# tvlearn/evo

Measured on AMD Instinct MI355X. Metric: E-step candidate-state evals/sec (NxS), full EM iteration, higher is better.
Workload: dtype f64; 1 GPU; ES3C D=256 H=512 S=200 N=100k f64 (north-star shape); algo=es3c, N_total=100000, N_rank0=100000, D=256, H=512, S=200, step=10 full EM iterations, world_size_rccl=1, ea=fit/randflip 10 parents x 1 child x 1 gen, states=p_init_Kn=1/H (init_states default), rng=device, mstep=device, parallelism=dp1

## Files before the change

### evo_amd/csrc/common.hpp

```cpp
#pragma once
#include <hip/hip_runtime.h>
#include <stdint.h>

typedef unsigned long long u64;
typedef long long i64;

#define EVO_F64_MIN (-1.7976931348623157e308)
#define EVO_F64_TINY (2.2250738585072014e-308)
#define EVO_WAVE 64

#define EVO_ERR_BAD_ENTRY 8
#define EVO_ERR_LIST_FULL 16
__device__ __forceinline__ int guard_index(int v, long long bound, int *__restrict__ err) {
  if (v < 0 || (long long)v >= bound) {
    atomicOr(err, EVO_ERR_BAD_ENTRY);
    return 0;
  }
  return v;
}
#define EVO_FLAG_NAN 1u
#define EVO_FLAG_NEGINF 2u
#define EVO_FLAG_POSINF 4u

__device__ __forceinline__ int wave_id_uniform() {
  return __builtin_amdgcn_readfirstlane((int)(threadIdx.x >> 6));
}
__device__ __forceinline__ int lane_id() { return (int)(threadIdx.x & 63); }

template <int CTRL, int ROWMASK>
__device__ __forceinline__ double dpp_move(double v) {
  const int lo = __double2loint(v), hi = __double2hiint(v);
  const int lo2 = __builtin_amdgcn_update_dpp(lo, lo, CTRL, ROWMASK, 0xF, false);
  const int hi2 = __builtin_amdgcn_update_dpp(hi, hi, CTRL, ROWMASK, 0xF, false);
  return __hiloint2double(hi2, lo2);
}
__device__ __forceinline__ double lane63_f64(double v) {
  const int lo = __builtin_amdgcn_readlane(__double2loint(v), 63);
  const int hi = __builtin_amdgcn_readlane(__double2hiint(v), 63);
  return __hiloint2double(hi, lo);
}
__device__ __forceinline__ double wave_sum(double v) {
  v += dpp_move<0xB1, 0xF>(v);
  v += dpp_move<0x4E, 0xF>(v);
  v += dpp_move<0x141, 0xF>(v);
  v += dpp_move<0x140, 0xF>(v);
  {
    const double t = dpp_move<0x142, 0xA>(v);
    if ((lane_id() >> 4) & 1) v += t;
  }
  {
    const double t = dpp_move<0x143, 0xC>(v);
    if (lane_id() >= 32) v += t;
  }
  return lane63_f64(v);
}
__device__ __forceinline__ double wave_max(double v) {
  v = fmax(v, dpp_move<0xB1, 0xF>(v));
  v = fmax(v, dpp_move<0x4E, 0xF>(v));
  v = fmax(v, dpp_move<0x141, 0xF>(v));
  v = fmax(v, dpp_move<0x140, 0xF>(v));
  v = fmax(v, dpp_move<0x142, 0xA>(v));
  v = fmax(v, dpp_move<0x143, 0xC>(v));
  return lane63_f64(v);
}
__device__ __forceinline__ unsigned dpp_max_u32(unsigned v, unsigned o) { return v > o ? v : o; }
template <int CTRL, int ROWMASK>
__device__ __forceinline__ unsigned dpp_move_u32(unsigned v) {
  return (unsigned)__builtin_amdgcn_update_dpp((int)v, (int)v, CTRL, ROWMASK, 0xF, false);
}
__device__ __forceinline__ unsigned row16_max_u32(unsigned v) {
  v = dpp_max_u32(v, dpp_move_u32<0xB1, 0xF>(v));
  v = dpp_max_u32(v, dpp_move_u32<0x4E, 0xF>(v));
  v = dpp_max_u32(v, dpp_move_u32<0x141, 0xF>(v));
  v = dpp_max_u32(v, dpp_move_u32<0x140, 0xF>(v));
  return v;
}
__device__ __forceinline__ unsigned wave_max_u32(unsigned v) {
  v = row16_max_u32(v);
  v = dpp_max_u32(v, dpp_move_u32<0x142, 0xA>(v));
  v = dpp_max_u32(v, dpp_move_u32<0x143, 0xC>(v));
  return (unsigned)__builtin_amdgcn_readlane((int)v, 63);
}

__device__ __forceinline__ unsigned wave_min_u32(unsigned v) { return ~wave_max_u32(~v); }
__device__ __forceinline__ double wave_min(double v);

__device__ __forceinline__ int wave_sum_i(int v) {
#pragma unroll
  for (int o = 32; o > 0; o >>= 1) v += __shfl_xor(v, o, 64);
  return v;
}

__device__ __forceinline__ double clamp_lpj(double v, unsigned &flags) {
  if (v != v) {
    flags |= EVO_FLAG_NAN;
    return EVO_F64_MIN;
  }
  if (isinf(v)) {
    flags |= (v < 0.0) ? EVO_FLAG_NEGINF : EVO_FLAG_POSINF;
    return 0.0;
  }
  return v;
}

__device__ __forceinline__ int pop_msb(u64 &bits) {
  int b = __clzll((long long)bits);
  bits &= ~(0x8000000000000000ull >> b);
  return b;
}

__device__ __forceinline__ double ordered_strided_sum(const double *__restrict__ p, i64 stride, i64 count) {
  double s = 0.0;
  i64 b = 0;
  for (; b + 8 <= count; b += 8) {
    double v[8];
#pragma unroll
    for (int u = 0; u < 8; u++) v[u] = p[(b + u) * stride];
#pragma unroll
    for (int u = 0; u < 8; u++) s += v[u];
  }
  for (; b < count; b++) s += p[b * stride];
  return s;
}

__device__ __forceinline__ void lds_barrier() { asm volatile("s_waitcnt lgkmcnt(0)\n\ts_barrier" ::: "memory"); }
__device__ __forceinline__ void lds_wave_fence() { asm volatile("s_waitcnt lgkmcnt(0)" ::: "memory"); }

#define DIG_IDX_BITS 14
#define DIG_MAX_H (1 << DIG_IDX_BITS)
#define DIG_SLOTS 4
__device__ __forceinline__ void digest_add(u64 &d, int &k, int h) {
  if (k < DIG_SLOTS) d |= (u64)h << (8 + DIG_IDX_BITS * k);
  k++;
}
__device__ __forceinline__ u64 digest_close(u64 d, int k) { return d | (u64)(k < 255 ? k : 255); }
__device__ __forceinline__ int dig_k(u64 d) { return (int)(d & 0xFFull); }
__device__ __forceinline__ int dig_idx(u64 d, int j) {
  return (int)((d >> (8 + DIG_IDX_BITS * j)) & (u64)(DIG_MAX_H - 1));
}
__device__ __forceinline__ u64 make_digest(const u64 *sp, int HW) {
  u64 d = 0;
  int k = 0;
  for (int w0 = 0; w0 < HW; w0 += 8) {
    u64 wv[8];
#pragma unroll
    for (int u = 0; u < 8; u++) wv[u] = (w0 + u < HW) ? sp[w0 + u] : 0ull;
#pragma unroll
    for (int u = 0; u < 8; u++) {
      u64 bits = wv[u];
      while (bits) digest_add(d, k, (w0 + u) * 64 + pop_msb(bits));
    }
  }
  return digest_close(d, k);
}

__device__ __forceinline__ double fast_rcp(double d) {
  double r = __builtin_amdgcn_rcp(d);
  r = fma(fma(-d, r, 1.0), r, r);
  r = fma(fma(-d, r, 1.0), r, r);
  return r;
}

struct LogDetAcc {
  double m = 1.0;
  int e = 0;
  __device__ __forceinline__ void mul(double d) {
    int ex;
    const double f = frexp(fabs(d), &ex);
    m *= f;
    e += ex;
    if (m < 0x1p-500) {
      int e2;
      m = frexp(m, &e2);
      e += e2;
    }
  }
  __device__ __forceinline__ double value() const { return log(m) + (double)e * 0.6931471805599453094; }
};

__device__ __forceinline__ double wave_max_dpp(double v) { return wave_max(v); }
__device__ __forceinline__ double wave_min(double v) { return -wave_max(-v); }
```

### evo_amd/csrc/evo_amd.hip

```cpp
#include "../../include/evo_amd.h"

#include <dlfcn.h>
#include <math.h>
#include <stdarg.h>
#include <stdio.h>
#include <stdlib.h>
#include <string.h>

#include <atomic>
#include <chrono>
#include <memory>
#include <string>
#include <type_traits>
#include <vector>

#include "common.hpp"
#include "gemm_f64.hpp"
#include "kernels_bsc.hpp"
#include "kernels_common.hpp"
#include "kernels_evolve.hpp"
#include "kernels_mstep.hpp"
#include "kernels_sssc.hpp"
#include "kernels_sssc_quad.hpp"
#include "kernels_fused.hpp"
// ... 343 lines not shown
  DevBuf<double> Y, yy, y2sum;
  int ldY = 0;
  PinnedBuf<double> h_acc, h_par;
  PinnedBuf<double> h_theta;
  double *h_theta_dev = nullptr;
  bool h_theta_fresh = false;
  DevBuf<double> theta_bak;
  bool theta_bak_valid = false;
  unsigned long long mbox_seq = 0;
  DevBuf<unsigned> mbox_counter;
  PinnedBuf<int> h_err;
  DevBuf<u64> states, cand;
  DevBuf<u64> dig, cand_dig;
  DevBuf<double> lpj, cand_lpj;
  DevBuf<double> lpj_alt;
  DevBuf<int> cand_counts;
  DevBuf<u64> cand_raw, dupold;
  DevBuf<int> gen_start;
  DevBuf<unsigned> flags;
  DevBuf<double> rowmax, rowsum, partial, partial2, diag;
  DevBuf<uint8_t> stage;
  DevBuf<double> W, Wt, G, Psi, Bm, mus, pilbar_v;
  DevBuf<double2> GP;
  DevBuf<double4> DG;
  DevBuf<double4> D1;
  DevBuf<PairEntry> PT;
  DevBuf<double> pies;
  double *dpar = nullptr;
  PinnedBuf<double> h_dpar;
  DevBuf<double> colpart;
  DevBuf<double> gjwork;
  DevBuf<double> tmpA, tmpB, tmpC;
  double ljc = 0;
  double *acc = nullptr;
  i64 acc_n = 0;
  DevBuf<double> acc_base;
  i64 ovf_n = 0;
  DevBuf<double> Es_own;
  double *Es = nullptr;
  DevBuf<int> list1, list2, list3, list_n, err;
  DevBuf<int> clist, clist_n;
  size_t clist_words() const { return clist.size() / 3; }
  DevBuf<OvfRec> ovf_rec;
  unsigned long long kn_gen = 1, census_gen = 0;
  int census_opt = 1;
  int merge_small = 1;
  DevBuf<double2> kap, cand_kap;
  unsigned long long kap_gen = ~0ull, cand_kap_gen = ~0ull;
  bool kap_carry = false;
  int stats_kappa = 1;
  int kappa_min = 16384;
  int stats_flat = 0;
  int fused_opt = 0;
  DevBuf<double> rowF;
  DevBuf<int> rowcnt, defer;
  DevBuf<double> fpart;
  DevBuf<unsigned long long> fprof;
  bool last_estep_fused = false;
  bool reduce_pending = false;
  long fused_calls = 0, unfused_calls = 0;
  int debug_poison_list = 0;
  int debug_fail_stats = 0;
  int census_skip = 0;
  DevBuf<double> tmp_y, tmp_lpj;
  DevBuf<u64> tmp_states;
  DevBuf<double> exact_buf;
  DevBuf<double> patch_img, patch_Y;
  DevBuf<double> patch_V;
  DevBuf<double> pred_buf, pred_Wt;
  DevBuf<int> pred_status;
  i64 pred_N = 0;
  int pred_D = 0;
  DevBuf<int> ps_slot, ps_status;
  DevBuf<u64> ps_s;
  DevBuf<double> ps_z, ps_y;
  i64 ps_N = 0, ps_T = 0;
  int ps_D = 0, ps_H = 0, ps_keep = -1;
  DevBuf<double> lle_d, lle_keep_d, lle_rho;
  DevBuf<int> lle_i;
  DevBuf<unsigned> lle_flags;
  DevBuf<u64> lle_keep_s, lle_hash;
  DevBuf<uint8_t> lle_keep_in;
  i64 lle_N = 0, lle_T = 0;
  int lle_H = 0, lle_keep = -1;
  DevBuf<uint8_t> codes_buf;
  unsigned long long rows_kn_gen = 0;
  int codes_path = -1;
  int init_home = -1;
  DevBuf<u64> init_scratch;
  DevBuf<double2> seed_gpt;
  DevBuf<double> seed_rows;
  DevBuf<double> refine_trace, score_buf;
  DevBuf<double> sweep_d;
  DevBuf<int> sweep_i;
  DevBuf<double> swap_d;
  DevBuf<int> swap_i;
  DevBuf<u64> remap_states, remap_dig;
  DevBuf<int> remap_i;
  DevBuf<unsigned long long> remap_sum, map_counts;
  i64 remap_N = 0;
  int remap_S = 0, remap_H = 0;
  DevBuf<u64> resize_states, resize_dig;
  DevBuf<int> resize_src;
  i64 resize_N = 0;
  int resize_S = 0, resize_H = 0;
  unsigned long long lpj_kn_gen = 0;
// ... 414 lines not shown
#define OPT_BOOL(f) nullptr, &evoamd_ctx::f
static int opt_flag(int v) { return v != 0; }
static const OptionRow OPTIONS[] = {
    {"sssc_k8", OPT_INT(k8_mode), [](int v) { return v < 0 ? -1 : (int)(v != 0); }},
    {"ebsc_f32", OPT_BOOL(f32_opt), opt_flag},
    {"bsc_direct", OPT_BOOL(bsc_direct), opt_flag, 0, 0, nullptr, nullptr,
     on_option_changes_derived},
    {"reconstruct_in_stats", OPT_BOOL(rec_in_stats), opt_flag},
    {"codes_path", OPT_INT(codes_path), nullptr, -1, CODES_GMEM, nullptr, "codes_path: -1 (auto), 0 registers, 1 LDS, 2 global memory"},
    {"merge_select_fused", OPT_INT(merge_select_fused), opt_flag},
    {"prefetch_lpj", OPT_BOOL(prefetch_lpj), opt_flag},
    {"inverse_block", OPT_INT(spd_block), nullptr, 0, 0, [](int v) { return v == 0 || v == 16 || v == 32; },
     "inverse_block: 0 (auto), 16 or 32"},
    {"overlap_gemm", OPT_INT(overlap_gemm)},
    {"stats_stage", OPT_INT(stats_stage)},
    {"stats_waves", OPT_INT(stats_waves)},
    {"pair_bins", OPT_INT(pair_bins)},
    {"gemm_streamk", OPT_INT(gemm_streamk)},
    {"b_transposed", OPT_INT(b_tn_opt)},
    {"pair_bins_scale", OPT_INT(bins_scale), nullptr, 1, 64, nullptr, "pair_bins_scale: 1 .. 64"},
    {"pair_bins_nwg", OPT_INT(bins_nwg), nullptr, 0, 0, [](int v) { return v >= 256 && v <= 2048 && (v % 256) == 0; },
     "pair_bins_nwg: 256 .. 2048, multiple of 256"},
    {"pair_bins_auto", OPT_INT(bins_auto), opt_flag},
    {"pair_bins_min", OPT_INT(bins_min)},
    {"bsc_stats_wave", OPT_INT(bsc_wave_opt)},
    {"gemm_workspace", OPT_INT(gemm_ws_opt)},
    {"sssc_precision", OPT_INT(sssc_prec32), [](int v) { return (int)(v == 32); }, 0, 0, [](int v) { return v == 64 || v == 32; },
     "sssc_precision: 64 or 32"},
    {"lpj_main_unstaged", OPT_INT(main_unstaged), opt_flag},
    {"lpj_singular_screen", OPT_INT(sing_screen), nullptr, 0, 2, nullptr, "lpj_singular_screen: 0 (never), 1 (automatic) or 2 (always)"},
    {"gemm_grouped", OPT_INT(gemm_grouped), opt_flag},
    {"gemm_per_xcd", OPT_INT(gemm_per_xcd)},
    {"init_states_home", OPT_INT(init_home), nullptr, -1, 1, nullptr, "init_states_home: -1 (auto), 0 LDS, 1 global memory"},
    {"background_unit", OPT_INT(bg_unit), opt_flag},
    {"fold_clear", OPT_INT(fold_clear), opt_flag},
    {"early_fork", OPT_INT(early_fork)},
    {"merge_small_levels", OPT_INT(merge_small), opt_flag},
    {"stats_flat", OPT_INT(stats_flat), opt_flag},
    {"theta_copy_engine", OPT_INT(theta_copy_engine), opt_flag},
    {"census_lists", OPT_INT(census_opt), opt_flag},
    {"sk_spare", OPT_INT(sk_spare), nullptr, -1, 32, nullptr, "sk_spare: -1 (automatic) or 0 .. 32 workgroups per XCD"},
    {"stats_chunks", OPT_INT(stats_chunks), nullptr, 1, 16, nullptr, "stats_chunks: 1 .. 16"},
    {"mailbox_side_stream", OPT_INT(mbox_side), opt_flag},
    {"fused_estep", OPT_INT(fused_opt), nullptr, 0, 2, nullptr, "fused_estep: 0 (never), 1 (automatic) or 2 (whenever the shape allows it)"},
    {"debug_poison_list", OPT_INT(debug_poison_list), opt_flag},
    {"debug_fail_stats", OPT_INT(debug_fail_stats), opt_flag},
    {"state_digest", OPT_BOOL(use_digest), opt_flag},
    {"inverse_spd", OPT_BOOL(spd_inverse), opt_flag},
};
static const OptionRow OPTIONS_LATER[] = {
  {"stats_kappa", OPT_INT(stats_kappa), nullptr, 0, 2, nullptr, "stats_kappa: 0 (never), 1 (automatic) or 2 (wherever the shape allows it)"},
  {"stats_kappa_min", OPT_INT(kappa_min), nullptr, 0, 1 << 20, nullptr, "stats_kappa_min: 0 .. 1048576 (x 1024 resident states)"},
};
#undef OPT_INT
#undef OPT_BOOL

extern "C" int evoamd_set_option(evoamd_ctx *c, const char *name, int value) {
  REQUIRE(c && name, "bad arguments");
  on_option(c);
  std::vector<const OptionRow *> rows;
  for (const OptionRow &o : OPTIONS) rows.push_back(&o);
  for (const OptionRow &o : OPTIONS_LATER) rows.push_back(&o);
  for (const OptionRow *row : rows) {
    const OptionRow &o = *row;
    if (strcmp(name, o.name) != 0) continue;
    if (o.err && !(o.accepts ? o.accepts(value) : (value >= o.lo && value <= o.hi))) return fail(EVOAMD_E_INVALID, "%s", o.err);
    const int v = o.norm ? o.norm(value) : value;
    if (o.ifield) c->*o.ifield = v;
    else c->*o.bfield = v != 0;
    if (o.after) o.after(c);
    return 0;
  }
  return fail(EVOAMD_E_INVALID, "unknown option '%s'", name);
}

static int join_fork(evoamd_ctx *c);

extern "C" int evoamd_synchronize(evoamd_ctx *c) {
  REQUIRE(c, "ctx is NULL");
  TRY(join_fork(c));
  HIP_TRY(hipStreamSynchronize(c->stream));
  return 0;
}

static i64 acc_len(const evoamd_ctx *c) {
  const i64 H = c->H, D = c->D;
  return (c->model == EVOAMD_MODEL_BSC) ? H * D + H * H + H + 1 + 8 : 2 * H + 4 * H * H + D * H + D + 8;
}
struct AccLayout {
  i64 Wp, Wq, pies, sigma;
  i64 xs, xss, xsz, xszsz, s_sz, sz_sz, sWp, y2;
  i64 tail;
};
static AccLayout acc_layout(const evoamd_ctx *c) {
  AccLayout a = {};
  const i64 H = c->H, D = c->D;
  if (c->model == EVOAMD_MODEL_BSC) {
    a.Wp = 0;
    a.Wq = H * D;
    a.pies = a.Wq + H * H;
    a.sigma = a.pies + H;
    a.tail = a.sigma + 1;
  } else {
    a.xs = 0;
    a.xss = H;
    a.xsz = a.xss + H * H;
    a.xszsz = a.xsz + H;
    a.sWp = a.xszsz + H * H;
    a.s_sz = a.sWp + D * H;
    a.sz_sz = a.s_sz + H * H;
    a.y2 = a.sz_sz + H * H;
    a.tail = a.y2 + D;
  }
  return a;
}
// ... 1594 lines not shown

extern "C" int evoamd_lpj_single_masked(evoamd_ctx *c, const double *y, const uint8_t *x_infr,
                                        const uint8_t *states_bool, int C, double *lpj_out, int32_t *flags_out) {
  REQUIRE(x_infr, "x_infr is NULL");
  return lpj_single_impl(c, y, x_infr, states_bool, C, lpj_out, flags_out);
}

static int estep_select(evoamd_ctx *c, int Mprime, double *sums_out) {
  on_kn_changed(c, KN_BY_SELECTION);
  {
    SpanGuard g(c, KID_VARY_KN);
    int *cl_n = census_mode(c) ? c->clist_n : nullptr;
    const i64 zero_n = c->fold_clear ? (i64)(c->ovf_n + c->acc_n) : 0;
    if (!c->fold_clear) cl_n = nullptr;
    const bool kap_carry = c->kap_carry && c->kap && c->cand_kap;
    with_spl(c->S, [&](auto spl) {
      with_cpl(c->Cmax, [&](auto cpl) {
        vary_kn_kernel<decltype(spl)::value, decltype(cpl)::value><<<cdiv(c->N, 4), 256, 0, c->stream>>>(
            c->states, c->lpj, c->cand, c->cand_lpj, c->cand_counts, c->N, c->S, c->S_perm, c->HW, c->Cmax, Mprime, c->rowmax,
            c->rowsum, c->partial, c->list_n, 4 * LIST_SHARDS, c->dig, c->cand_dig, (c->use_digest && c->dig) ? 1 : 0,
            c->pending_skip, c->err, cl_n, 4 * LIST_SHARDS, c->census_skip, c->acc_base, zero_n,
            kap_carry ? c->kap.get() : nullptr, kap_carry ? c->cand_kap.get() : nullptr);
      });
    });
    reduce3_partials_kernel<<<1, R3_THREADS, 0, c->stream>>>(c->partial, cdiv(c->N, 4), c->dpar);
    HIP_TRY(hipGetLastError());
    DBG_SYNC(c, "vary_kn");
    made_selection(c, cl_n != nullptr, zero_n > 0, kap_carry);
  }
  if (sums_out) {
    HIP_TRY(hipMemcpyAsync(sums_out, c->dpar + DP_ECNT0, 2 * sizeof(double), hipMemcpyDeviceToHost, c->stream));
    HIP_TRY(hipStreamSynchronize(c->stream));
  }
  return 0;
}

extern "C" int evoamd_vary_kn(evoamd_ctx *c, int Mprime, double *sums_out) {
  REQUIRE(c && c->configured && c->have_cand, "no resident candidate batch (call lpj_candidates / evolve first)");
  TRY(estep_check_mprime(c, Mprime));
  REQUIRE_KN(c);
  HIP_TRY(hipSetDevice(c->device));
  return estep_select(c, Mprime, sums_out);
}

extern "C" int evoamd_set_estep_counts(evoamd_ctx *c, double sum_nunique, double sum_sub) {
  REQUIRE(c && c->configured, "configure first");
  HIP_TRY(hipSetDevice(c->device));
  double v[2] = {sum_nunique, sum_sub};
  HIP_TRY(hipMemcpyAsync(c->dpar + DP_ECNT0, v, sizeof(v), hipMemcpyHostToDevice, c->stream));
  HIP_TRY(hipStreamSynchronize(c->stream));
  return 0;
}

static int estep_children(evoamd_ctx *c, int n_parents, int n_children, uint64_t seed, int fit_parents) {
  {
    SpanGuard g(c, KID_EVOLVE);
    with_spl(c->S, [&](auto spl) {
      evolve_randflip_kernel<decltype(spl)::value><<<cdiv(c->N, 4), 256, 0, c->stream>>>(
          c->states, c->lpj, c->N, c->S, c->S_perm, c->H - c->bg_unit, c->HW, n_parents, n_children, c->Cmax, seed, fit_parents,
          c->cand, c->cand_counts, c->list_n, c->model == EVOAMD_MODEL_SSSC ? 4 * LIST_SHARDS : 0, c->cand_dig, c->pending_skip,
          c->err);
    });
    HIP_TRY(hipGetLastError());
    DBG_SYNC(c, "evolve");
    made_clean_lists(c);
    on_cand_installed(c, true);
  }
  TRY(eval_candidates(c));
  made_cand_lpj(c);
  return 0;
}

extern "C" int evoamd_evolve_randflip(evoamd_ctx *c, int n_parents, int n_children, uint64_t seed, int fit_parents) {
  TRY(estep_check_randflip(c, n_parents, n_children));
  REQUIRE_KN(c);
  HIP_TRY(hipSetDevice(c->device));
  return estep_children(c, n_parents, n_children, seed, fit_parents);
}

static bool fused_shape_ok(const evoamd_ctx *c, int n_parents, int n_children) {
  return c->model == EVOAMD_MODEL_SSSC && c->S_perm == 0 && !c->bg_unit && !c->mask_infr && c->use_digest && c->dig && census_mode(c) &&
         c->H <= 1024 && c->H >= 2 && (c->H % 2) == 0 && n_parents * n_children <= 64 && n_parents * n_children <= c->Cmax &&
         c->rowF && c->defer &&
         ((size_t)(1024 / c->S + 2) * c->H + (c->H <= 512 ? (size_t)4 * c->H : 0)) * sizeof(double) <= MAIN_LPJ_LDS_MAX;
}

#define FUSED_LDS_MAX (150 * 1024)
static const i64 INKERNEL_CENSUS_BELOW = (i64)4 << 20;

struct FusedStage {
  int W, kc_big, lds_wave_bytes;
  size_t lds;
  unsigned grid;
};
struct EstepPlan {
  bool fused = false;
  int spl = 1;
  bool inkernel_census = false;
  FusedStage st[2] = {};
};

static int estep_plan(const evoamd_ctx *c, int n_parents, int n_children, EstepPlan &p) {
  p = EstepPlan{};
  with_spl(c->S, [&](auto spl) { p.spl = decltype(spl)::value; });
  p.fused = c->fused_opt != 0 && fused_shape_ok(c, n_parents, n_children);
  if (p.fused && c->fused_opt == 1) p.fused = c->need_known && c->res_cnt[1] <= 0.25 * (double)c->N;
  if (!p.fused) return 0;
  p.inkernel_census = c->N * (i64)c->S < INKERNEL_CENSUS_BELOW;
  const size_t tab = (size_t)4 * c->H * sizeof(double);
  for (int stage = 0; stage < 2; stage++) {
    FusedStage &st = p.st[stage];
    st.W = stage == 0 ? 4 : 1;
    st.kc_big = stage == 0 ? 16 : SSSC_KCAP;
    st.lds_wave_bytes = fused_lds_wave_bytes(p.spl, st.kc_big);
// ... 3314 lines not shown
```

### evo_amd/csrc/kernels_evolve.hpp

```cpp
#pragma once
#include "common.hpp"
#include "kernels_common.hpp"

__device__ __forceinline__ u64 mix64(u64 x) {
  x ^= x >> 30;
  x *= 0xbf58476d1ce4e5b9ull;
  x ^= x >> 27;
  x *= 0x94d049bb133111ebull;
  x ^= x >> 31;
  return x;
}
__device__ __forceinline__ double rng_u01(u64 seed, u64 n, u64 purpose, u64 index) {
  u64 x = mix64(seed + 0x9e3779b97f4a7c15ull * (n + 1));
  x = mix64(x ^ (purpose * 0xd1b54a32d192ed03ull + index + 0x632be59bd9b4e019ull));
  return ((double)(x >> 11) + 0.5) * (1.0 / 9007199254740992.0);
}

#define EV_MAX_S_PER_LANE 16
#define EV_MAX_CHILDREN 8

template <int SPL>
__global__ __launch_bounds__(256) void evolve_randflip_kernel(
    const u64 *__restrict__ states, const double *__restrict__ lpj, i64 N, int S, int S_perm, int H, int HW,
    int n_parents, int n_children, int Cmax, u64 seed, int fit_parents, u64 *__restrict__ cand,
    int *__restrict__ counts, int *__restrict__ list_n, int n_list, u64 *__restrict__ cand_dig, int skipped_mask,
    int *__restrict__ err) {
  __shared__ int sel_sh[4][64];
  if (blockIdx.x == 0 && list_n)
    clear_lists_checked(list_n, n_list, skipped_mask, err);
  const int lane = lane_id(), wave = wave_id_uniform();
  const i64 n = (i64)blockIdx.x * 4 + wave;
  if (n >= N) return;
  int *sel = sel_sh[wave];
  const double *row = lpj + n * (S + S_perm) + S_perm;
  double key[SPL];
  double lmin = INFINITY;
#pragma unroll
  for (int q = 0; q < SPL; q++) {
    int s = lane + 64 * q;
    key[q] = (s < S) ? row[s] : INFINITY;
    lmin = fmin(lmin, key[q]);
  }
  lmin = wave_min(lmin);
  const double shift = 2.0 * fmin(lmin, 0.0);
  constexpr unsigned KEY_TAKEN = 0x7f800000u;
  unsigned ukey[SPL];
#pragma unroll
  for (int q = 0; q < SPL; q++) {
    int s = lane + 64 * q;
    unsigned k = KEY_TAKEN;
    if (s < S) {
      const double p = fit_parents ? (key[q] - shift) : 1.0;
      const double u = rng_u01(seed, (u64)n, 1, (u64)s);
      const float uf = fmaxf((float)u, 1.17549435e-38f);
      const float lg = __logf(uf);
      const float e = lg < 0.0f ? -lg : 0.0f;
      float kf = 1e30f;
      if (p > 0.0) kf = fminf(__fdividef(e, (float)p), 3.0e38f);
      k = __float_as_uint(kf);
    }
    ukey[q] = k;
  }
  for (int j = 0; j < n_parents; j++) {
    unsigned bv = ukey[0];
#pragma unroll
    for (int q = 1; q < SPL; q++) bv = ukey[q] < bv ? ukey[q] : bv;
    const unsigned gv = wave_min_u32(bv);
    int bi = 0x7fffffff;
#pragma unroll
    for (int q = 0; q < SPL; q++) {
      const u64 hit = __ballot(ukey[q] == gv);
      if (bi == 0x7fffffff && hit != 0ull) bi = 64 * q + __ffsll((long long)hit) - 1;
    }
    if (lane == 0) sel[j] = bi;
    if ((bi & 63) == lane) {
#pragma unroll
      for (int q = 0; q < SPL; q++)
        if (q == (bi >> 6)) ukey[q] = KEY_TAKEN;
    }
  }
  __builtin_amdgcn_wave_barrier();
  __threadfence_block();
  const int n_kids = n_parents * n_children;
  for (int kid = lane; kid < n_kids; kid += 64) {
    const int p = kid / n_children, i = kid - p * n_children;
    int picks[EV_MAX_CHILDREN];
    int mine = 0;
    for (int t = 0; t <= i; t++) {
      int r = (int)(rng_u01(seed, (u64)n, 2 + (u64)p, (u64)t) * (double)(H - t));
      if (r >= H - t) r = H - t - 1;
      int pos = 0;
      for (int t2 = 0; t2 < t; t2++)
        if (picks[t2] <= r) {
          r++;
          pos = t2 + 1;
        }
      for (int t2 = t; t2 > pos; t2--) picks[t2] = picks[t2 - 1];
      picks[pos] = r;
      mine = r;
    }
    const u64 *par = states + (n * (i64)S + sel[p]) * HW;
    u64 *dst = cand + (n * (i64)Cmax + kid) * HW;
    u64 d = 0;
    int dk = 0;
    for (int w0 = 0; w0 < HW; w0 += 8) {
      u64 pv[8];
#pragma unroll
      for (int u = 0; u < 8; u++) pv[u] = (w0 + u < HW) ? par[w0 + u] : 0ull;
#pragma unroll
      for (int u = 0; u < 8; u++) {
        const int w = w0 + u;
        if (w < HW) {
          u64 v = pv[u];
          if (w == (mine >> 6)) v ^= (0x8000000000000000ull >> (mine & 63));
          dst[w] = v;
          while (v) digest_add(d, dk, w * 64 + pop_msb(v));
        }
      }
    }
    if (cand_dig) cand_dig[n * (i64)Cmax + kid] = digest_close(d, dk);
  }
  if (lane == 0) counts[n] = n_kids;
}

enum { EV_RANDFLIP = 0, EV_SPARSEFLIP = 1, EV_CROSS = 2, EV_CROSS_RANDFLIP = 3, EV_CROSS_SPARSEFLIP = 4 };

#define EVG_MAX_S 1024
#define EVG_MAX_C 256
#define EVG_POOL (EVG_MAX_S + EVG_MAX_C)
#define EVG_FLAGW ((1 + EVG_MAX_S + EVG_MAX_C + 63) / 64)

struct EvolveArgs {
  const u64 *states;
  const u64 *dig;
  const double *lpj;
  u64 *cand;
  u64 *cand_dig;
  const double *cand_lpj;
  u64 *raw;
  int *counts;
  int *gen_start;
  u64 *dupold;
  i64 N;
  int S, S_perm, H, HW, Cmax;
  int gen, n_parents, n_children, kind, fit_parents;
  u64 seed;
  double sparseness, p_bf;
};

__device__ __forceinline__ const u64 *evg_state(const EvolveArgs &a, i64 n, int u) {
  const int j = u - a.S_perm;
  return j < a.S ? a.states + (n * (i64)a.S + j) * a.HW : a.cand + (n * (i64)a.Cmax + (j - a.S)) * a.HW;
}

__device__ __forceinline__ u64 evg_domain_mask(int w, int H) {
  const int valid = H - 64 * w;
  return valid >= 64 ? ~0ull : (valid <= 0 ? 0ull : (~0ull << (64 - valid)));
}

__device__ __forceinline__ void evg_sparse_p(double H, double s_abs, double sparseness, double p_bf, double &p0, double &p1) {
  const double eps = 1e-100;
  const double alpha = (H - s_abs) * ((H * p_bf) - (sparseness - s_abs)) / ((sparseness - s_abs + H * p_bf) * s_abs + eps);
  p0 = (H * p_bf) / (H + (alpha - 1.0) * s_abs + eps);
  p1 = alpha * p0;
}

__global__ __launch_bounds__(64) void evolve_general_kernel(EvolveArgs a) {
  __shared__ u64 ksig[EVG_MAX_S];
  __shared__ u64 csig[EVG_MAX_C];
  __shared__ u64 rsig[EVG_MAX_C];
  __shared__ int pool_u[EVG_POOL];
  __shared__ double pool_f[EVG_POOL];
  __shared__ unsigned pool_key[EVG_POOL];
// ... 278 lines not shown
```

### evo_amd/csrc/kernels_fused.hpp

```cpp
#pragma once
#include "kernels_evolve.hpp"
#include "kernels_sssc_quad.hpp"

struct FusedArgs {
  SsscArgs a;
  u64 *states;
  u64 *dig;
  double *lpj;
  int S, n_parents, n_children, fit_parents, Mprime;
  u64 seed;
  double *rowmax, *rowsum, *rowF;
  int *rowcnt;
  unsigned *flags_res, *flags_cand;
  const int *in_items, *in_count;
  int *out_items, *out_count;
  int list_cap;
  int stage_d1;
  int *cen_items, *cen_n;
  i64 cen_stride;
  int cen_cap;
  u64 *cand;
  int Cmax;
  int kc_big;
  int lds_wave_bytes;
  unsigned long long *prof;
};
#ifdef FUSED_PROFILE
#define FPROF(slot)                                                                    \
  do {                                                                                 \
    const unsigned long long _t = __builtin_readcyclecounter();                        \
    _pacc[slot] += _t - _tp;    \
    _tp = _t;                                                                          \
  } while (0)
#else
#define FPROF(slot) do {} while (0)
#endif

__device__ __forceinline__ u64 digest_toggle(const u64 pd, const int h) {
  const int k = dig_k(pd);
  constexpr int INF = 0x7fffffff;
  const int l0 = k > 0 ? dig_idx(pd, 0) : INF, l1 = k > 1 ? dig_idx(pd, 1) : INF, l2 = k > 2 ? dig_idx(pd, 2) : INF,
            l3 = k > 3 ? dig_idx(pd, 3) : INF;
  const bool e0 = l0 == h, e1 = l1 == h, e2 = l2 == h, e3 = l3 == h;
  int n0, n1, n2, n3, nk;
  if (e0 || e1 || e2 || e3) {
    n0 = e0 ? l1 : l0;
    n1 = (e0 || e1) ? l2 : l1;
    n2 = (e0 || e1 || e2) ? l3 : l2;
    n3 = INF;
    nk = k - 1;
  } else {
    n0 = min(l0, h);
    const int r0 = max(l0, h);
    n1 = min(l1, r0);
    const int r1 = max(l1, r0);
    n2 = min(l2, r1);
    const int r2 = max(l2, r1);
    n3 = min(l3, r2);
    nk = k + 1;
  }
  u64 d = (u64)nk;
  if (nk > 0) d |= (u64)n0 << (8 + DIG_IDX_BITS * 0);
  if (nk > 1) d |= (u64)n1 << (8 + DIG_IDX_BITS * 1);
  if (nk > 2) d |= (u64)n2 << (8 + DIG_IDX_BITS * 2);
  if (nk > 3) d |= (u64)n3 << (8 + DIG_IDX_BITS * 3);
  return d;
}

__device__ __forceinline__ u64 digest_word(const u64 d, const int w) {
  const int k = dig_k(d);
  u64 v = 0ull;
#pragma unroll
  for (int j = 0; j < DIG_SLOTS; j++) {
    const int h = dig_idx(d, j);
    if (j < k && (h >> 6) == w) v |= 0x8000000000000000ull >> (h & 63);
  }
  return v;
}

__device__ __forceinline__ void vm_wave_fence() { asm volatile("s_waitcnt vmcnt(0)" ::: "memory"); }
__device__ __forceinline__ u64 load_sc0(const u64 *p) {
  return __hip_atomic_load(p, __ATOMIC_RELAXED, __HIP_MEMORY_SCOPE_WORKGROUP);
}

__host__ __device__ inline int fused_lds_wave_bytes(int SPL, int kc_big) {
  int b = SPL * 64 * 8 * 2;
  b += 64 * 8 * 3;
  b += 64 * 2 * 2;
  b += 64 * 4 * 3;
  b += 32 * 4;
  b += (16 * 8 + 16) * 4;
  b += (4 * kc_big * kc_big + 5 * kc_big) * 8 + ((kc_big * 4 + 7) / 8) * 8;
  return (b + 15) / 16 * 16;
}

template <int SPL, bool LISTED>
__global__ __launch_bounds__(256, 2) void sssc_estep_fused_kernel(FusedArgs f) {
  SsscArgs &a = f.a;
  a.s2inv = a.dpar[DP_S2INV];
  extern __shared__ double fsm[];
  constexpr int SP = SPL * 64;
  const int H = a.H, HW = a.HW, S = f.S;
  const int lane = lane_id(), wave = wave_id_uniform(), W = (int)(blockDim.x >> 6);
  const i64 count = LISTED ? (i64)min(*f.in_count, f.list_cap) : a.N;
  if (LISTED && count == 0) return;
  double4 *d1s = (double4 *)fsm;
  char *wb = (char *)(fsm + (f.stage_d1 ? (size_t)4 * H : 0)) + (size_t)wave * f.lds_wave_bytes;
  double *rowL = (double *)wb;
  u64 *rowD = (u64 *)(rowL + SP);
  u64 *cdig = rowD + SP;
  double *cval = (double *)(cdig + 64);
  double *new_v = cval + 64;
  unsigned short *lst = (unsigned short *)(new_v + 64);
  unsigned short *hlst = lst + 64;
  int *sel = (int *)(hlst + 64);
  int *new_i = sel + 64, *old_i = new_i + 64;
  int *dbuf = old_i + 64;
  int *idxb = dbuf + 32;
  int *kcnt = idxb + 16 * 8;
  BigLds BL;
  BL.carve((double *)(kcnt + 16), f.kc_big);
  if (f.stage_d1) {
    for (int i = threadIdx.x; i < H; i += blockDim.x) d1s[i] = a.D1[i];
    __syncthreads();
  }
  const double4 *D1t = f.stage_d1 ? d1s : a.D1;
  const bool exact = sssc_exact_mode(a);
  const double s2 = a.s2inv;
  const int n_kids = f.n_parents * f.n_children;
  const u64 lt_mask = (1ull << lane) - 1ull;
  const int t4 = lane & 3, qd = lane >> 2;
// ... 538 lines not shown
```

Before: 5.120 billion state evals/s.

## Add lean randflip evolve kernel with sorted parent race and digest toggling

Adds a lean evolve kernel that is on by default when HW < 4096. It presorts each lane's race keys so parent selection needs one wave-min per parent, and picks the flip index directly when there is one child. It derives the candidate digest by toggling the parent's digest instead of rescanning the state bits. Candidate words are written as a flat, coalesced (kid, word) copy using magic-number division. Dedicated DPP min/max helpers replace the complement-based min. The aim is to cut per-state scalar work and uncoalesced writes in the evolve step, at the cost of more kernel code and an extra LDS array.

```diff
diff --git a/evo_amd/csrc/common.hpp b/evo_amd/csrc/common.hpp
--- a/evo_amd/csrc/common.hpp
+++ b/evo_amd/csrc/common.hpp
@@ -63,26 +63,39 @@
   v = fmax(v, dpp_move<0x143, 0xC>(v));
   return lane63_f64(v);
 }
-__device__ __forceinline__ unsigned dpp_max_u32(unsigned v, unsigned o) { return v > o ? v : o; }
 template <int CTRL, int ROWMASK>
-__device__ __forceinline__ unsigned dpp_move_u32(unsigned v) {
-  return (unsigned)__builtin_amdgcn_update_dpp((int)v, (int)v, CTRL, ROWMASK, 0xF, false);
+__device__ __forceinline__ unsigned dpp_max_u32(unsigned v) {
+  const unsigned o = (unsigned)__builtin_amdgcn_update_dpp(0, (int)v, CTRL, ROWMASK, 0xF, false);
+  return v > o ? v : o;
+}
+template <int CTRL, int ROWMASK>
+__device__ __forceinline__ unsigned dpp_min_u32(unsigned v) {
+  const unsigned o = (unsigned)__builtin_amdgcn_update_dpp(-1, (int)v, CTRL, ROWMASK, 0xF, false);
+  return v < o ? v : o;
 }
 __device__ __forceinline__ unsigned row16_max_u32(unsigned v) {
-  v = dpp_max_u32(v, dpp_move_u32<0xB1, 0xF>(v));
-  v = dpp_max_u32(v, dpp_move_u32<0x4E, 0xF>(v));
-  v = dpp_max_u32(v, dpp_move_u32<0x141, 0xF>(v));
-  v = dpp_max_u32(v, dpp_move_u32<0x140, 0xF>(v));
+  v = dpp_max_u32<0xB1, 0xF>(v);
+  v = dpp_max_u32<0x4E, 0xF>(v);
+  v = dpp_max_u32<0x141, 0xF>(v);
+  v = dpp_max_u32<0x140, 0xF>(v);
   return v;
 }
 __device__ __forceinline__ unsigned wave_max_u32(unsigned v) {
   v = row16_max_u32(v);
-  v = dpp_max_u32(v, dpp_move_u32<0x142, 0xA>(v));
-  v = dpp_max_u32(v, dpp_move_u32<0x143, 0xC>(v));
+  v = dpp_max_u32<0x142, 0xA>(v);
+  v = dpp_max_u32<0x143, 0xC>(v);
   return (unsigned)__builtin_amdgcn_readlane((int)v, 63);
 }
 
-__device__ __forceinline__ unsigned wave_min_u32(unsigned v) { return ~wave_max_u32(~v); }
+__device__ __forceinline__ unsigned wave_min_u32(unsigned v) {
+  v = dpp_min_u32<0xB1, 0xF>(v);
+  v = dpp_min_u32<0x4E, 0xF>(v);
+  v = dpp_min_u32<0x141, 0xF>(v);
+  v = dpp_min_u32<0x140, 0xF>(v);
+  v = dpp_min_u32<0x142, 0xA>(v);
+  v = dpp_min_u32<0x143, 0xC>(v);
+  return (unsigned)__builtin_amdgcn_readlane((int)v, 63);
+}
 __device__ __forceinline__ double wave_min(double v);
 
 __device__ __forceinline__ int wave_sum_i(int v) {
@@ -152,6 +165,48 @@
     }
   }
   return digest_close(d, k);
+}
+
+__device__ __forceinline__ u64 digest_toggle(const u64 pd, const int h) {
+  const int k = dig_k(pd);
+  constexpr int INF = 0x7fffffff;
+  const int l0 = k > 0 ? dig_idx(pd, 0) : INF, l1 = k > 1 ? dig_idx(pd, 1) : INF, l2 = k > 2 ? dig_idx(pd, 2) : INF,
+            l3 = k > 3 ? dig_idx(pd, 3) : INF;
+  const bool e0 = l0 == h, e1 = l1 == h, e2 = l2 == h, e3 = l3 == h;
+  int n0, n1, n2, n3, nk;
+  if (e0 || e1 || e2 || e3) {
+    n0 = e0 ? l1 : l0;
+    n1 = (e0 || e1) ? l2 : l1;
+    n2 = (e0 || e1 || e2) ? l3 : l2;
+    n3 = INF;
+    nk = k - 1;
+  } else {
+    n0 = min(l0, h);
+    const int r0 = max(l0, h);
+    n1 = min(l1, r0);
+    const int r1 = max(l1, r0);
+    n2 = min(l2, r1);
+    const int r2 = max(l2, r1);
+    n3 = min(l3, r2);
+    nk = k + 1;
+  }
+  u64 d = (u64)nk;
+  if (nk > 0) d |= (u64)n0 << (8 + DIG_IDX_BITS * 0);
+  if (nk > 1) d |= (u64)n1 << (8 + DIG_IDX_BITS * 1);
+  if (nk > 2) d |= (u64)n2 << (8 + DIG_IDX_BITS * 2);
+  if (nk > 3) d |= (u64)n3 << (8 + DIG_IDX_BITS * 3);
+  return d;
+}
+
+__device__ __forceinline__ u64 digest_word(const u64 d, const int w) {
+  const int k = dig_k(d);
+  u64 v = 0ull;
+#pragma unroll
+  for (int j = 0; j < DIG_SLOTS; j++) {
+    const int h = dig_idx(d, j);
+    if (j < k && (h >> 6) == w) v |= 0x8000000000000000ull >> (h & 63);
+  }
+  return v;
 }
 
 __device__ __forceinline__ double fast_rcp(double d) {
diff --git a/evo_amd/csrc/evo_amd.hip b/evo_amd/csrc/evo_amd.hip
--- a/evo_amd/csrc/evo_amd.hip
+++ b/evo_amd/csrc/evo_amd.hip
@@ -419,6 +419,7 @@
   int kappa_min = 16384;
   int stats_flat = 0;
   int fused_opt = 0;
+  int evolve_lean = -1;
   DevBuf<double> rowF;
   DevBuf<int> rowcnt, defer;
   DevBuf<double> fpart;
@@ -939,6 +940,9 @@
   {"stats_kappa", OPT_INT(stats_kappa), nullptr, 0, 2, nullptr, "stats_kappa: 0 (never), 1 (automatic) or 2 (wherever the shape allows it)"},
   {"stats_kappa_min", OPT_INT(kappa_min), nullptr, 0, 1 << 20, nullptr, "stats_kappa_min: 0 .. 1048576 (x 1024 resident states)"},
 };
+static const OptionRow OPTIONS_ESTEP[] = {
+  {"evolve_lean", OPT_INT(evolve_lean), nullptr, -1, 1, nullptr, "evolve_lean: -1 (automatic), 0 or 1"},
+};
 #undef OPT_INT
 #undef OPT_BOOL
 
@@ -948,6 +952,7 @@
   std::vector<const OptionRow *> rows;
   for (const OptionRow &o : OPTIONS) rows.push_back(&o);
   for (const OptionRow &o : OPTIONS_LATER) rows.push_back(&o);
+  for (const OptionRow &o : OPTIONS_ESTEP) rows.push_back(&o);
   for (const OptionRow *row : rows) {
     const OptionRow &o = *row;
     if (strcmp(name, o.name) != 0) continue;
@@ -2648,14 +2653,24 @@
   return 0;
 }
 
+static unsigned magic_of(int d) { return d == 1 ? 0u : (unsigned)(0x100000000ull / (unsigned)d + 1ull); }
+static bool evolve_lean_ok(const evoamd_ctx *c) { return c->HW < 4096; }
+static bool evolve_lean_on(const evoamd_ctx *c) { return c->evolve_lean != 0 && evolve_lean_ok(c); }
+
 static int estep_children(evoamd_ctx *c, int n_parents, int n_children, uint64_t seed, int fit_parents) {
   {
     SpanGuard g(c, KID_EVOLVE);
+    const int n_list = c->model == EVOAMD_MODEL_SSSC ? 4 * LIST_SHARDS : 0;
     with_spl(c->S, [&](auto spl) {
-      evolve_randflip_kernel<decltype(spl)::value><<<cdiv(c->N, 4), 256, 0, c->stream>>>(
-          c->states, c->lpj, c->N, c->S, c->S_perm, c->H - c->bg_unit, c->HW, n_parents, n_children, c->Cmax, seed, fit_parents,
-          c->cand, c->cand_counts, c->list_n, c->model == EVOAMD_MODEL_SSSC ? 4 * LIST_SHARDS : 0, c->cand_dig, c->pending_skip,
-          c->err);
+      if (evolve_lean_on(c))
+        evolve_randflip_lean_kernel<decltype(spl)::value><<<cdiv(c->N, 4), 256, 0, c->stream>>>(
+            c->states, c->use_digest ? c->dig.get() : nullptr, c->lpj, c->N, c->S, c->S_perm, c->H - c->bg_unit, c->HW, n_parents,
+            n_children, c->Cmax, seed, fit_parents, c->cand, c->cand_counts, c->list_n, n_list, c->cand_dig, c->pending_skip,
+            c->err, magic_of(c->HW), magic_of(n_children));
+      else
+        evolve_randflip_kernel<decltype(spl)::value><<<cdiv(c->N, 4), 256, 0, c->stream>>>(
+            c->states, c->lpj, c->N, c->S, c->S_perm, c->H - c->bg_unit, c->HW, n_parents, n_children, c->Cmax, seed, fit_parents,
+            c->cand, c->cand_counts, c->list_n, n_list, c->cand_dig, c->pending_skip, c->err);
     });
     HIP_TRY(hipGetLastError());
     DBG_SYNC(c, "evolve");
diff --git a/evo_amd/csrc/kernels_evolve.hpp b/evo_amd/csrc/kernels_evolve.hpp
--- a/evo_amd/csrc/kernels_evolve.hpp
+++ b/evo_amd/csrc/kernels_evolve.hpp
@@ -18,6 +18,58 @@
 
 #define EV_MAX_S_PER_LANE 16
 #define EV_MAX_CHILDREN 8
+
+constexpr unsigned EV_KEY_TAKEN = 0x7f800000u;
+template <int SPL>
+__device__ __forceinline__ void ev_race_keys(const double *__restrict__ row, int S, i64 n, u64 seed, int fit_parents,
+                                             unsigned (&ukey)[SPL]) {
+  const int lane = lane_id();
+  double key[SPL];
+  double lmin = INFINITY;
+#pragma unroll
+  for (int q = 0; q < SPL; q++) {
+    int s = lane + 64 * q;
+    key[q] = (s < S) ? row[s] : INFINITY;
+    lmin = fmin(lmin, key[q]);
+  }
+  lmin = wave_min(lmin);
+  const double shift = 2.0 * fmin(lmin, 0.0);
+#pragma unroll
+  for (int q = 0; q < SPL; q++) {
+    int s = lane + 64 * q;
+    unsigned k = EV_KEY_TAKEN;
+    if (s < S) {
+      const double p = fit_parents ? (key[q] - shift) : 1.0;
+      const double u = rng_u01(seed, (u64)n, 1, (u64)s);
+      const float uf = fmaxf((float)u, 1.17549435e-38f);
+      const float lg = __logf(uf);
+      const float e = lg < 0.0f ? -lg : 0.0f;
+      float kf = 1e30f;
+      if (p > 0.0) kf = fminf(__fdividef(e, (float)p), 3.0e38f);
+      k = __float_as_uint(kf);
+    }
+    ukey[q] = k;
+  }
+}
+
+__device__ __forceinline__ int ev_pick(u64 seed, i64 n, int p, int i, int H) {
+  int picks[EV_MAX_CHILDREN];
+  int mine = 0;
+  for (int t = 0; t <= i; t++) {
+    int r = (int)(rng_u01(seed, (u64)n, 2 + (u64)p, (u64)t) * (double)(H - t));
+    if (r >= H - t) r = H - t - 1;
+    int pos = 0;
+    for (int t2 = 0; t2 < t; t2++)
+      if (picks[t2] <= r) {
+        r++;
+        pos = t2 + 1;
+      }
+    for (int t2 = t; t2 > pos; t2--) picks[t2] = picks[t2 - 1];
+    picks[pos] = r;
+    mine = r;
+  }
+  return mine;
+}
 
 template <int SPL>
 __global__ __launch_bounds__(256) void evolve_randflip_kernel(
@@ -33,34 +85,9 @@
   if (n >= N) return;
   int *sel = sel_sh[wave];
   const double *row = lpj + n * (S + S_perm) + S_perm;
-  double key[SPL];
-  double lmin = INFINITY;
-#pragma unroll
-  for (int q = 0; q < SPL; q++) {
-    int s = lane + 64 * q;
-    key[q] = (s < S) ? row[s] : INFINITY;
-    lmin = fmin(lmin, key[q]);
-  }
-  lmin = wave_min(lmin);
-  const double shift = 2.0 * fmin(lmin, 0.0);
-  constexpr unsigned KEY_TAKEN = 0x7f800000u;
+  constexpr unsigned KEY_TAKEN = EV_KEY_TAKEN;
   unsigned ukey[SPL];
-#pragma unroll
-  for (int q = 0; q < SPL; q++) {
-    int s = lane + 64 * q;
-    unsigned k = KEY_TAKEN;
-    if (s < S) {
-      const double p = fit_parents ? (key[q] - shift) : 1.0;
-      const double u = rng_u01(seed, (u64)n, 1, (u64)s);
-      const float uf = fmaxf((float)u, 1.17549435e-38f);
-      const float lg = __logf(uf);
-      const float e = lg < 0.0f ? -lg : 0.0f;
-      float kf = 1e30f;
-      if (p > 0.0) kf = fminf(__fdividef(e, (float)p), 3.0e38f);
-      k = __float_as_uint(kf);
-    }
-    ukey[q] = k;
-  }
+  ev_race_keys<SPL>(row, S, n, seed, fit_parents, ukey);
   for (int j = 0; j < n_parents; j++) {
     unsigned bv = ukey[0];
 #pragma unroll
@@ -84,21 +111,7 @@
   const int n_kids = n_parents * n_children;
   for (int kid = lane; kid < n_kids; kid += 64) {
     const int p = kid / n_children, i = kid - p * n_children;
-    int picks[EV_MAX_CHILDREN];
-    int mine = 0;
-    for (int t = 0; t <= i; t++) {
-      int r = (int)(rng_u01(seed, (u64)n, 2 + (u64)p, (u64)t) * (double)(H - t));
-      if (r >= H - t) r = H - t - 1;
-      int pos = 0;
-      for (int t2 = 0; t2 < t; t2++)
-        if (picks[t2] <= r) {
-          r++;
-          pos = t2 + 1;
-        }
-      for (int t2 = t; t2 > pos; t2--) picks[t2] = picks[t2 - 1];
-      picks[pos] = r;
-      mine = r;
-    }
+    const int mine = ev_pick(seed, n, p, i, H);
     const u64 *par = states + (n * (i64)S + sel[p]) * HW;
     u64 *dst = cand + (n * (i64)Cmax + kid) * HW;
     u64 d = 0;
@@ -119,6 +132,143 @@
       }
     }
     if (cand_dig) cand_dig[n * (i64)Cmax + kid] = digest_close(d, dk);
+  }
+  if (lane == 0) counts[n] = n_kids;
+}
+
+__device__ __forceinline__ int magic_div(int t, int d, unsigned magic) { return d == 1 ? t : (int)__umulhi((unsigned)t, magic); }
+
+template <int SPL>
+__global__ __launch_bounds__(256) void evolve_randflip_lean_kernel(
+    const u64 *__restrict__ states, const u64 *__restrict__ dig, const double *__restrict__ lpj, i64 N, int S, int S_perm,
+    int H, int HW, int n_parents, int n_children, int Cmax, u64 seed, int fit_parents, u64 *__restrict__ cand,
+    int *__restrict__ counts, int *__restrict__ list_n, int n_list, u64 *__restrict__ cand_dig, int skipped_mask,
+    int *__restrict__ err, unsigned magic_hw, unsigned magic_nc) {
+  constexpr bool SORTED = SPL <= 4;
+  __shared__ int sel_sh[4][64];
+  __shared__ int flip_sh[4][64 * VK_MAX_C_PER_LANE];
+  if (blockIdx.x == 0 && list_n)
+    clear_lists_checked(list_n, n_list, skipped_mask, err);
+  const int lane = lane_id(), wave = wave_id_uniform();
+  const i64 n = (i64)blockIdx.x * 4 + wave;
+  if (n >= N) return;
+  int *sel = sel_sh[wave], *flip = flip_sh[wave];
+  const double *row = lpj + n * (S + S_perm) + S_perm;
+  constexpr unsigned KEY_TAKEN = EV_KEY_TAKEN;
+  unsigned ukey[SPL];
+  ev_race_keys<SPL>(row, S, n, seed, fit_parents, ukey);
+  if constexpr (SORTED) {
+    unsigned sq[SPL];
+#pragma unroll
+    for (int q = 0; q < SPL; q++) sq[q] = (unsigned)q;
+#pragma unroll
+    for (int ph = 0; ph < SPL; ph++) {
+#pragma unroll
+      for (int a = ph & 1; a + 1 < SPL; a += 2) {
+        const bool sw = ukey[a + 1] < ukey[a];
+        const unsigned klo = sw ? ukey[a + 1] : ukey[a], khi = sw ? ukey[a] : ukey[a + 1];
+        const unsigned qlo = sw ? sq[a + 1] : sq[a], qhi = sw ? sq[a] : sq[a + 1];
+        ukey[a] = klo, ukey[a + 1] = khi;
+        sq[a] = qlo, sq[a + 1] = qhi;
+      }
+    }
+    unsigned perm = 0;
+#pragma unroll
+    for (int q = 0; q < SPL; q++) perm |= sq[q] << (2 * q);
+    for (int j = 0; j < n_parents; j++) {
+      const unsigned gv = wave_min_u32(ukey[0]);
+      int bi = 0;
+      if (gv != KEY_TAKEN) {
+        const u64 hit = __ballot(ukey[0] == gv);
+        const unsigned idx = (unsigned)lane + 64u * (perm & 3u);
+        if (hit & (hit - 1ull))
+          bi = (int)wave_min_u32(ukey[0] == gv ? idx : 0xFFFFFFFFu);
+        else
+          bi = __builtin_amdgcn_readlane((int)idx, __ffsll((long long)hit) - 1);
+        if ((bi & 63) == lane) {
+#pragma unroll
+          for (int q = 0; q + 1 < SPL; q++) ukey[q] = ukey[q + 1];
+          ukey[SPL - 1] = KEY_TAKEN;
+          perm >>= 2;
+        }
+      }
+      if (lane == 0) sel[j] = bi;
+    }
+  } else {
+    for (int j = 0; j < n_parents; j++) {
+      unsigned bv = ukey[0];
+#pragma unroll
+      for (int q = 1; q < SPL; q++) bv = ukey[q] < bv ? ukey[q] : bv;
+      const unsigned gv = wave_min_u32(bv);
+      int bi = 0x7fffffff;
+#pragma unroll
+      for (int q = 0; q < SPL; q++) {
+        const u64 hit = __ballot(ukey[q] == gv);
+        if (bi == 0x7fffffff && hit != 0ull) bi = 64 * q + __ffsll((long long)hit) - 1;
+      }
+      if (lane == 0) sel[j] = bi;
+      if ((bi & 63) == lane) {
+#pragma unroll
+        for (int q = 0; q < SPL; q++)
+          if (q == (bi >> 6)) ukey[q] = KEY_TAKEN;
+      }
+    }
+  }
+  __builtin_amdgcn_wave_barrier();
+  __threadfence_block();
+  const int n_kids = n_parents * n_children;
+  const u64 *st_n = states + n * (i64)S * HW;
+  for (int kid = lane; kid < n_kids; kid += 64) {
+    const int p = magic_div(kid, n_children, magic_nc), i = kid - p * n_children;
+    const int ps = sel[p];
+    u64 pd = 0;
+    if (dig && cand_dig) pd = dig[n * (i64)S + ps];
+    int mine;
+    if (n_children == 1) {
+      mine = (int)(rng_u01(seed, (u64)n, 2 + (u64)p, 0) * (double)H);
+      if (mine >= H) mine = H - 1;
+    } else {
+      mine = ev_pick(seed, n, p, i, H);
+    }
+    flip[kid] = mine;
+    if (cand_dig) {
+      u64 cd;
+      if (dig && dig_k(pd) <= DIG_SLOTS) {
+        cd = digest_toggle(pd, mine);
+      } else {
+        const u64 *par = st_n + (i64)ps * HW;
+        u64 d = 0;
+        int dk = 0;
+        for (int w = 0; w < HW; w++) {
+          u64 v = par[w];
+          if (w == (mine >> 6)) v ^= (0x8000000000000000ull >> (mine & 63));
+          while (v) digest_add(d, dk, w * 64 + pop_msb(v));
+        }
+        cd = digest_close(d, dk);
+      }
+      cand_dig[n * (i64)Cmax + kid] = cd;
+    }
+  }
+  __builtin_amdgcn_wave_barrier();
+  __threadfence_block();
+  const int n_pairs = n_kids * HW;
+  u64 *cd_n = cand + n * (i64)Cmax * HW;
+  for (int t0 = lane; t0 < n_pairs; t0 += 128) {
+    u64 v[2];
+#pragma unroll
+    for (int u = 0; u < 2; u++) {
+      const int t = t0 + 64 * u;
+      v[u] = 0ull;
+      if (t < n_pairs) {
+        const int kid = magic_div(t, HW, magic_hw), w = t - kid * HW;
+        const int mine = flip[kid];
+        v[u] = st_n[(i64)sel[magic_div(kid, n_children, magic_nc)] * HW + w];
+        if (w == (mine >> 6)) v[u] ^= (0x8000000000000000ull >> (mine & 63));
+      }
+    }
+#pragma unroll
+    for (int u = 0; u < 2; u++)
+      if (t0 + 64 * u < n_pairs) cd_n[t0 + 64 * u] = v[u];
   }
   if (lane == 0) counts[n] = n_kids;
 }
diff --git a/evo_amd/csrc/kernels_fused.hpp b/evo_amd/csrc/kernels_fused.hpp
--- a/evo_amd/csrc/kernels_fused.hpp
+++ b/evo_amd/csrc/kernels_fused.hpp
@@ -35,48 +35,6 @@
 #else
 #define FPROF(slot) do {} while (0)
 #endif
-
-__device__ __forceinline__ u64 digest_toggle(const u64 pd, const int h) {
-  const int k = dig_k(pd);
-  constexpr int INF = 0x7fffffff;
-  const int l0 = k > 0 ? dig_idx(pd, 0) : INF, l1 = k > 1 ? dig_idx(pd, 1) : INF, l2 = k > 2 ? dig_idx(pd, 2) : INF,
-            l3 = k > 3 ? dig_idx(pd, 3) : INF;
-  const bool e0 = l0 == h, e1 = l1 == h, e2 = l2 == h, e3 = l3 == h;
-  int n0, n1, n2, n3, nk;
-  if (e0 || e1 || e2 || e3) {
-    n0 = e0 ? l1 : l0;
-    n1 = (e0 || e1) ? l2 : l1;
-    n2 = (e0 || e1 || e2) ? l3 : l2;
-    n3 = INF;
-    nk = k - 1;
-  } else {
-    n0 = min(l0, h);
-    const int r0 = max(l0, h);
-    n1 = min(l1, r0);
-    const int r1 = max(l1, r0);
-    n2 = min(l2, r1);
-    const int r2 = max(l2, r1);
-    n3 = min(l3, r2);
-    nk = k + 1;
-  }
-  u64 d = (u64)nk;
-  if (nk > 0) d |= (u64)n0 << (8 + DIG_IDX_BITS * 0);
-  if (nk > 1) d |= (u64)n1 << (8 + DIG_IDX_BITS * 1);
-  if (nk > 2) d |= (u64)n2 << (8 + DIG_IDX_BITS * 2);
-  if (nk > 3) d |= (u64)n3 << (8 + DIG_IDX_BITS * 3);
-  return d;
-}
-
-__device__ __forceinline__ u64 digest_word(const u64 d, const int w) {
-  const int k = dig_k(d);
-  u64 v = 0ull;
-#pragma unroll
-  for (int j = 0; j < DIG_SLOTS; j++) {
-    const int h = dig_idx(d, j);
-    if (j < k && (h >> 6) == w) v |= 0x8000000000000000ull >> (h & 63);
-  }
-  return v;
-}
 
 __device__ __forceinline__ void vm_wave_fence() { asm volatile("s_waitcnt vmcnt(0)" ::: "memory"); }
 __device__ __forceinline__ u64 load_sc0(const u64 *p) {
```

New measurement: 5.146 billion state evals/s (median of 6 runs). About the same (+0.5%).
